# rosariocannavo/testudo

Hardware: AMD Instinct MI355X
Metric: PST commit+open sec, 2^20-var poly BLS12-377; G1 MSM Mscalar/s at 1/2/4/8 GPU (higher is better)
Workload: dtype u32; 1 GPU; single BLS12-377 G1 Pippenger MSM, 2^20 points per GPU (BASELINE configs[1]); n_points=1048576, curve=BLS12-377 G1, window_bits=16, parallelism=1 GPU

## Files before the change

### testudo_amd/csrc/msm_batch.hip

```cpp
#include "msm_sort.h"
#include "msm_acc.h"
#include "msm_reduce.h"

namespace tpst {

__global__ void __launch_bounds__(64, 1) k_build_tables(const uint32_t* __restrict__ bases, size_t N, int c, int W, uint32_t* __restrict__ table) {
  const size_t j = (size_t)blockIdx.x * blockDim.x + threadIdx.x;
  if (j >= N) return;
  G1A p = load_affine<Fq>(bases, j);
  for (int w = 0; w < W; w++) {
    store_rec29(table, (size_t)w * N + j, p);
    if (w + 1 < W) {
      Xyzz<Fq> x = to_xyzz(p);
      for (int i = 0; i < c; i++) x = dbl(x);
      p = to_affine(x);
    }
  }
}

hipError_t batch_tables_build(hipStream_t s, const uint32_t* d_bases, size_t N, int c, BatchTables& t) {
  batch_tables_free(t);
  t.N = N;
  t.c = c;
  t.W = num_windows(c);
  TPST_TRY(hipMalloc(&t.d_table, (size_t)t.W * N * REC29_WORDS * sizeof(uint32_t)));
  k_build_tables<<<grid_for(N, 64), 64, 0, s>>>(d_bases, N, c, t.W, t.d_table);
  return hipGetLastError();
}

void batch_tables_free(BatchTables& t) {
  if (t.d_table) (void)hipFree(t.d_table);
  t.d_table = nullptr;
  t.N = 0;
}

__device__ __forceinline__ void zero_bucket(uint4* zb, size_t key) {
  constexpr int Q = sizeof(Xyzz<Fq>) / 16;
#pragma unroll
  for (int i = 0; i < Q; i++) zb[key * Q + i] = make_uint4(0, 0, 0, 0);
}

__global__ void __launch_bounds__(256) k_batch_sort(const uint32_t* __restrict__ scalars, size_t rows, size_t N,
                                                    size_t row_stride, size_t col_stride, int c, int W,
                                                    uint32_t* __restrict__ keys, uint32_t* __restrict__ entries,
                                                    uint32_t* __restrict__ bstart, uint32_t* __restrict__ bend,
                                                    uint4* __restrict__ zb) {
  extern __shared__ uint32_t cnt[];
  const size_t nblk = gridDim.x;
  size_t r = blockIdx.x;
  if (nblk % 8 == 0) r = (blockIdx.x % 8) * (nblk / 8) + blockIdx.x / 8;
  if (r >= rows) return;
  const uint32_t nb = 1u << (c - 1);
  for (uint32_t b = threadIdx.x; b < nb; b += blockDim.x) cnt[b] = 0;
  __syncthreads();
  for (size_t j = threadIdx.x; j < N; j += blockDim.x) {
    uint32_t s[8];
    load_scalar(scalars + 8 * (r * row_stride + j * col_stride), s);
    uint32_t carry = 0;
    for (int w = 0; w < W; w++) {
      const int d = signed_digit(s, 8, w, c, W, carry);
      if (d) atomicAdd(&cnt[abs(d) - 1], 1u);
    }
  }
  __syncthreads();
  __shared__ uint32_t part[256];
  __shared__ uint32_t total_sh;
  const uint32_t per = (nb + blockDim.x - 1) / blockDim.x;
  const uint32_t b0 = threadIdx.x * per;
  uint32_t local = 0;
  for (uint32_t b = b0; b < b0 + per && b < nb; b++) local += cnt[b];
  part[threadIdx.x] = local;
  __syncthreads();
  if (threadIdx.x == 0) {
    uint32_t run = 0;
    for (unsigned t = 0; t < blockDim.x; t++) {
      const uint32_t v = part[t];
      part[t] = run;
      run += v;
    }
    total_sh = run;
  }
  __syncthreads();
  const size_t rowbase = r * N * (size_t)W;
  uint32_t run = part[threadIdx.x];
  for (uint32_t b = b0; b < b0 + per && b < nb; b++) {
    const uint32_t v = cnt[b];
    if (!v) zero_bucket(zb, r * nb + b);
    bstart[r * nb + b] = (uint32_t)(rowbase + run);
    bend[r * nb + b] = (uint32_t)(rowbase + run + v);
    cnt[b] = run;
    run += v;
  }
  __syncthreads();
  for (size_t j = threadIdx.x; j < N; j += blockDim.x) {
    uint32_t s[8];
    load_scalar(scalars + 8 * (r * row_stride + j * col_stride), s);
    uint32_t carry = 0;
    for (int w = 0; w < W; w++) {
      const int d = signed_digit(s, 8, w, c, W, carry);
      if (d) {
        const uint32_t b = (uint32_t)abs(d) - 1;
        const uint32_t pos = atomicAdd(&cnt[b], 1u);
        keys[rowbase + pos] = (uint32_t)(r * nb + b);
        entries[rowbase + pos] = (uint32_t)(w * N + j) | (d < 0 ? 0x80000000u : 0u);
      }
    }
  }
  const uint32_t total = total_sh;
  const uint32_t sent = (uint32_t)(rows * nb);
  for (size_t e = total + threadIdx.x; e < N * (size_t)W; e += blockDim.x) keys[rowbase + e] = sent;
}

constexpr int SB_THREADS = 1024;
constexpr int SB_SPT = 4;
constexpr uint32_t SB_NB = 2048;
constexpr uint32_t SB_STAGE = 15 * 1024;

template <int WC, int CC = 12>
__global__ void __launch_bounds__(SB_THREADS) k_batch_sort_staged(const uint32_t* __restrict__ scalars, size_t rows,
                                                                 size_t N, size_t row_stride, size_t col_stride, int c,
                                                                 int W, uint32_t* __restrict__ keys,
                                                                 uint32_t* __restrict__ entries,
                                                                 uint32_t* __restrict__ bstart,
                                                                 uint32_t* __restrict__ bend,
                                                                 uint4* __restrict__ zb) {
  __shared__ uint32_t start[SB_NB + 1];
  __shared__ uint32_t cur[SB_NB];
  __shared__ uint2 stage[SB_STAGE];
  __shared__ uint32_t part[SB_THREADS / 64];
  __shared__ uint32_t pass_lo, pass_hi;
  const size_t nblk = gridDim.x;
  size_t r = blockIdx.x;
  if (nblk % 8 == 0) r = (blockIdx.x % 8) * (nblk / 8) + blockIdx.x / 8;
  if (r >= rows) return;
  const uint32_t nb = 1u << (c - 1);
  const int tid = threadIdx.x;
  for (uint32_t b = tid; b < nb; b += SB_THREADS) cur[b] = 0;
  __syncthreads();
  for (int k = 0; k < SB_SPT; k++) {
    const size_t j = (size_t)tid + (size_t)k * SB_THREADS;
    if (j >= N) break;
    uint32_t sc[8];
    load_scalar(scalars + 8 * (r * row_stride + j * col_stride), sc);
    uint32_t carry = 0;
    if constexpr (WC > 0) {
#pragma unroll
      for (int w = 0; w < WC; w++) {
        const int d = signed_digit(sc, 8, w, CC, WC, carry);
        if (d) atomicAdd(&cur[abs(d) - 1], 1u);
      }
    } else {
      for (int w = 0; w < W; w++) {
        const int d = signed_digit(sc, 8, w, c, W, carry);
        if (d) atomicAdd(&cur[abs(d) - 1], 1u);
      }
    }
  }
  __syncthreads();
  {
    const uint32_t per = (nb + SB_THREADS - 1) / SB_THREADS;
    const uint32_t b0 = tid * per;
    uint32_t local = 0;
    for (uint32_t b = b0; b < b0 + per && b < nb; b++) local += cur[b];
    const int lane = tid & 63, wv = tid >> 6;
    uint32_t incl = local;
    for (int o = 1; o < 64; o <<= 1) {
      const uint32_t v = __shfl_up(incl, o, 64);
      if (lane >= o) incl += v;
    }
    if (lane == 63) part[wv] = incl;
    __syncthreads();
    if (tid == 0) {
      uint32_t run = 0;
      for (int i = 0; i < SB_THREADS / 64; i++) {
        const uint32_t v = part[i];
        part[i] = run;
        run += v;
      }
      start[nb] = run;
    }
    __syncthreads();
    uint32_t run = part[wv] + incl - local;
    for (uint32_t b = b0; b < b0 + per && b < nb; b++) {
      const uint32_t v = cur[b];
      start[b] = run;
      run += v;
    }
  }
  __syncthreads();
  const size_t rowbase = r * N * (size_t)W;
  for (uint32_t b = tid; b < nb; b += SB_THREADS) {
    if (start[b + 1] == start[b]) zero_bucket(zb, r * nb + b);
    bstart[r * nb + b] = (uint32_t)(rowbase + start[b]);
    bend[r * nb + b] = (uint32_t)(rowbase + start[b + 1]);
    cur[b] = start[b];
  }
  const uint32_t total = start[nb];
  if (tid == 0) pass_hi = 0;
  __syncthreads();
  for (;;) {
    if (tid == 0) {
      const uint32_t lo = pass_hi;
      uint32_t hi = lo;
      if (lo < nb) {
        const uint32_t lim = start[lo] + SB_STAGE;
        uint32_t a = lo + 1, z = nb;
        while (a < z) {
          const uint32_t m = (a + z + 1) >> 1;
          if (start[m] <= lim) a = m; else z = m - 1;
        }
        hi = a;
      }
      pass_lo = lo;
      pass_hi = hi;
    }
    __syncthreads();
    const uint32_t lo = pass_lo, hi = pass_hi;
    if (lo >= nb) break;
    const uint32_t p0 = start[lo], cnt = start[hi] - p0;
    const bool direct = cnt > SB_STAGE;
    auto place = [&](int d, int w, size_t j) {
      if (!d) return;
      const uint32_t b = (uint32_t)abs(d) - 1;
      if (b < lo || b >= hi) return;
      const uint32_t pos = atomicAdd(&cur[b], 1u);
      const uint2 e = make_uint2((uint32_t)(r * nb + b), (uint32_t)(w * N + j) | (d < 0 ? 0x80000000u : 0u));
      if (direct) {
        keys[rowbase + pos] = e.x;
        entries[rowbase + pos] = e.y;
      } else {
        stage[pos - p0] = e;
      }
    };
    for (int k = 0; k < SB_SPT; k++) {
      const size_t j = (size_t)tid + (size_t)k * SB_THREADS;
      if (j >= N) break;
      uint32_t sc[8];
      load_scalar(scalars + 8 * (r * row_stride + j * col_stride), sc);
      uint32_t carry = 0;
      if constexpr (WC > 0) {
#pragma unroll
        for (int w = 0; w < WC; w++) place(signed_digit(sc, 8, w, CC, WC, carry), w, j);
      } else {
        for (int w = 0; w < W; w++) place(signed_digit(sc, 8, w, c, W, carry), w, j);
      }
    }
    __syncthreads();
    if (!direct) {
      for (uint32_t i = tid; i < cnt; i += SB_THREADS) {
        const uint2 e = stage[i];
        keys[rowbase + p0 + i] = e.x;
        entries[rowbase + p0 + i] = e.y;
      }
    }
    __syncthreads();
  }
  const uint32_t sent = (uint32_t)(rows * nb);
  for (size_t e = total + tid; e < N * (size_t)W; e += SB_THREADS) keys[rowbase + e] = sent;
}

hipError_t msm_batch(Arena& ar, hipStream_t s, const BatchTables& t, const uint32_t* d_scalars, size_t rows,
                     size_t row_stride, size_t col_stride, Xyzz<Fq>* d_out) {
  if (rows == 0) return hipSuccess;
  const int c = t.c, W = t.W;
  const size_t N = t.N;
  const uint32_t nb = 1u << (c - 1);
  const size_t m = rows * N * (size_t)W;
  if (m >= (1ull << 32)) return hipErrorInvalidValue;
  const size_t nbk = rows * nb;
  static const size_t k1_threads = (size_t)4 * 64 * device_simds();
  int lg = 5;
  while (lg < 8 && (m >> (lg + 1)) >= k1_threads) lg++;
  const size_t nchunk = (m + ((size_t)1 << lg) - 1) >> lg;
  const size_t nblk = (nchunk + ACC_BLOCK - 1) / ACC_BLOCK;
  size_t need = 2 * Arena::need(m, 4) + 2 * Arena::need(nbk, 4) + Arena::need(nbk, sizeof(Xyzz<Fq>)) +
                Arena::need(nchunk, sizeof(Xyzz<Fq>)) + Arena::need(nblk, sizeof(Xyzz<Fq>)) +
                reduce_scratch<Fq>(rows, nb) + (red2_ok(nb) ? reduce2_scratch<Fq>(rows, nb) : 0) + 4096;
  ar.reset();
  TPST_TRY(ar.reserve(need));
  uint32_t* keys = ar.take<uint32_t>(m);
  uint32_t* entries = ar.take<uint32_t>(m);
  Xyzz<Fq>* part = ar.take<Xyzz<Fq>>(nchunk);
  Xyzz<Fq>* bpart = ar.take<Xyzz<Fq>>(nblk);
  uint32_t* bstart = ar.take<uint32_t>(nbk);
  uint32_t* bend = ar.take<uint32_t>(nbk);
  Xyzz<Fq>* buckets = ar.take<Xyzz<Fq>>(nbk);
  const unsigned nrow_blk = (unsigned)rows;
  Profiler* pf = ar.prof;
  Profiler dummy;
  if (!pf) pf = &dummy;
  pf->begin(ST_BATCH_SORT, s);
  if (N <= (size_t)SB_THREADS * SB_SPT && c == 12 && W == 22)
    k_batch_sort_staged<22, 12><<<nrow_blk, SB_THREADS, 0, s>>>(d_scalars, rows, N, row_stride, col_stride, c, W, keys,
                                                                 entries, bstart, bend, reinterpret_cast<uint4*>(buckets));
  else if (N <= (size_t)SB_THREADS * SB_SPT && c == 11 && W == 24)
    k_batch_sort_staged<24, 11><<<nrow_blk, SB_THREADS, 0, s>>>(d_scalars, rows, N, row_stride, col_stride, c, W, keys,
                                                                 entries, bstart, bend, reinterpret_cast<uint4*>(buckets));
  else if (N <= (size_t)SB_THREADS * SB_SPT && nb <= SB_NB)
    k_batch_sort_staged<0><<<nrow_blk, SB_THREADS, 0, s>>>(d_scalars, rows, N, row_stride, col_stride, c, W, keys,
                                                            entries, bstart, bend, reinterpret_cast<uint4*>(buckets));
  else
    k_batch_sort<<<nrow_blk, 256, nb * sizeof(uint32_t), s>>>(d_scalars, rows, N, row_stride, col_stride, c, W, keys,
                                                          entries, bstart, bend, reinterpret_cast<uint4*>(buckets));
  TPST_TRY(hipGetLastError());
  pf->end(ST_BATCH_SORT, s);
  pf->begin(ST_BUCKET_ACC, s);
  k_bucket_acc_chunk_lds<TPST_K1_MINW><<<(unsigned)nblk, ACC_BLOCK, 0, s>>>(keys, entries, m, nullptr, (uint32_t)nbk, bstart, bend,
                                                                  t.d_table, lg, buckets, part, bpart);
  TPST_TRY(hipGetLastError());
  k_bucket_fixup<Fq><<<grid_for(nblk, 64), 64, 0, s>>>(keys, m, nullptr, (uint32_t)nbk, bstart, bend, lg, nblk,
                                                       part, bpart, buckets);
  TPST_TRY(hipGetLastError());
  pf->end(ST_BUCKET_ACC, s);
  pf->begin(ST_REDUCE, s);
  if (red2_ok(nb))
    TPST_TRY(reduce_buckets2<Fq>(ar, s, buckets, rows, nb, d_out, 0));
  else
    TPST_TRY(reduce_buckets<Fq>(ar, s, buckets, rows, nb, d_out));
  pf->end(ST_REDUCE, s);
  return hipSuccess;
}

}
```

### testudo_amd/csrc/msm_reduce.h

```cpp
#pragma once
#include "msm_common.h"

namespace tpst {

template <bool PK, class F>
__device__ __forceinline__ Xyzz<typename AccField<F>::T> load_in(const Xyzz<F>* p, size_t i) {
  if constexpr (PK)
    return load_pk(p, i);
  else
    return load_acc(p, i);
}

template <class F, bool PK>
__global__ void __launch_bounds__(64) k_seg_reduce_quad(const Xyzz<F>* __restrict__ buckets, uint32_t nb, uint32_t L,
                                                        size_t nseg, Xyzz<F>* __restrict__ seg_out, int prio = 0) {
  using C = typename AccField<F>::T;
  set_wave_prio(prio);
  const size_t t = ((size_t)blockIdx.x * blockDim.x + threadIdx.x) >> 2;
  const int qi = threadIdx.x & 3;
  if (t >= nseg) return;
  const uint32_t S = nb / L;
  const size_t g = t / S;
  const uint32_t k = (uint32_t)(t % S);
  const size_t base = g * nb + (size_t)k * L;
  Xyzz<C> acc = Xyzz<C>::inf(), sum = Xyzz<C>::inf();
  for (int b = (int)L - 1; b >= 0; b--) {
    acc = add_quad(acc, load_in<PK>(buckets, base + b), qi);
    sum = add_quad(sum, acc, qi);
  }
  const uint32_t s0 = k * L;
  if (s0 != 0 && !is_inf(acc)) sum = add_quad(sum, scalar_mul_quad(acc, s0, 32 - __builtin_clz(s0), qi), qi);
  if (qi == 0) store_acc(seg_out, t, sum);
}

template <class F, bool PK>
__global__ void __launch_bounds__(64) k_seg_reduce_lane(const Xyzz<F>* __restrict__ buckets, uint32_t nb, uint32_t L,
                                                        size_t nseg, Xyzz<F>* __restrict__ seg_out) {
  using C = typename AccField<F>::T;
  const size_t t = (size_t)blockIdx.x * blockDim.x + threadIdx.x;
  if (t >= nseg) return;
  const uint32_t S = nb / L;
  const size_t g = t / S;
  const uint32_t k = (uint32_t)(t % S);
  const size_t base = g * nb + (size_t)k * L;
  Xyzz<C> acc = Xyzz<C>::inf(), sum = Xyzz<C>::inf();
  for (int b = (int)L - 1; b >= 0; b--) {
    acc = add(acc, load_in<PK>(buckets, base + b));
    sum = add(sum, acc);
  }
  const uint32_t s0 = k * L;
  if (s0 != 0 && !is_inf(acc)) sum = add(sum, scalar_mul_xyzz(acc, &s0, 32 - __builtin_clz(s0)));
  store_acc(seg_out, t, sum);
}

template <class F, int BS>
__global__ void __launch_bounds__(BS) k_group_reduce_quad(const Xyzz<F>* __restrict__ seg, uint32_t S,
                                                          Xyzz<F>* __restrict__ out, int prio = 0) {
  using C = typename AccField<F>::T;
  set_wave_prio(prio);
  constexpr int Q = BS / 4;
  __shared__ Xyzz<C> sh[Q];
  const size_t g = blockIdx.x;
  const int quad = threadIdx.x >> 2, qi = threadIdx.x & 3;
  Xyzz<C> acc = Xyzz<C>::inf();
  for (uint32_t k = quad; k < S; k += Q) acc = add_quad(acc, load_acc(seg, g * S + k), qi);
  if (qi == 0) sh[quad] = acc;
  __syncthreads();
  for (int h = Q / 2; h > 0; h >>= 1) {
    if (quad < h) {
      const Xyzz<C> v = add_quad(sh[quad], sh[quad + h], qi);
      if (qi == 0) sh[quad] = v;
    }
    __syncthreads();
  }
  if (threadIdx.x == 0) store_acc(out, g, sh[0]);
}

template <class F>
static __global__ void __launch_bounds__(64, 1) k_window_chain(const Xyzz<F>* __restrict__ win, int wlo, int whi,
                                                              int c, const Xyzz<F>* __restrict__ extra, int nextra,
                                                              Xyzz<F>* __restrict__ out) {
  using C = typename AccField<F>::T;
  if (blockIdx.x != 0) return;
  __builtin_amdgcn_s_setprio(3);
  const int qi = threadIdx.x & 3;
  Xyzz<C> acc = load_acc(win, whi - 1);
  for (int w = whi - 2; w >= wlo; w--) {
    for (int i = 0; i < c; i++) acc = dbl_quad(acc, qi);
    acc = add_quad(acc, load_acc(win, w), qi);
  }
  for (int i = 0; i < c * wlo; i++) acc = dbl_quad(acc, qi);
  for (int k = 0; k < nextra; k++) acc = add_quad(acc, load_acc(extra, k), qi);
  if (threadIdx.x == 0) store_acc(out, 0, acc);
}

static uint32_t reduce_seg_len(size_t groups, uint32_t nb) {
  uint32_t L = 4;
  while (L < 32 && 2 * L <= nb && groups * (nb / (2 * L)) >= ((size_t)1 << 18)) L *= 2;
  return nb >= L ? L : nb;
}

template <class F>
static size_t reduce_scratch(size_t groups, uint32_t nb) {
  const uint32_t L = reduce_seg_len(groups, nb);
  const size_t nseg = groups * (nb / L);
  return Arena::need(nseg, sizeof(Xyzz<F>)) + Arena::need(nseg / 64 + groups + 1, sizeof(Xyzz<F>));
}

template <class F>
static hipError_t sum_groups(Arena& ar, hipStream_t s, const Xyzz<F>* in, size_t groups, uint32_t S, Xyzz<F>* out,
                             int prio) {
  if (S >= 256 && S % 64 == 0) {
    Xyzz<F>* mid = ar.take<Xyzz<F>>(groups * S / 64);
    k_group_reduce_quad<F, 256><<<(unsigned)(groups * S / 64), 256, 0, s>>>(in, 64, mid, prio);
    TPST_TRY(hipGetLastError());
    k_group_reduce_quad<F, 256><<<(unsigned)groups, 256, 0, s>>>(mid, S / 64, out, prio);
  } else {
    k_group_reduce_quad<F, 256><<<(unsigned)groups, 256, 0, s>>>(in, S, out, prio);
  }
  return hipGetLastError();
}

template <class F>
static hipError_t reduce_buckets(Arena& ar, hipStream_t s, const Xyzz<F>* d_buckets, size_t groups, uint32_t nb,
                                 Xyzz<F>* d_group_out, int prio = 0, bool pk = true) {
  const uint32_t L = reduce_seg_len(groups, nb);
  const uint32_t S = nb / L;
  const size_t nseg = groups * S;
  Xyzz<F>* seg = ar.take<Xyzz<F>>(nseg);
  if (std::is_same<F, Fq>::value && nseg >= ((size_t)1 << 18)) {
    if (pk)
      k_seg_reduce_lane<F, true><<<grid_for(nseg, 64), 64, 0, s>>>(d_buckets, nb, L, nseg, seg);
    else
      k_seg_reduce_lane<F, false><<<grid_for(nseg, 64), 64, 0, s>>>(d_buckets, nb, L, nseg, seg);
  } else if (pk) {
    k_seg_reduce_quad<F, true><<<grid_for(4 * nseg, 64), 64, 0, s>>>(d_buckets, nb, L, nseg, seg, prio);
  } else {
    k_seg_reduce_quad<F, false><<<grid_for(4 * nseg, 64), 64, 0, s>>>(d_buckets, nb, L, nseg, seg, prio);
  }
  TPST_TRY(hipGetLastError());
  return sum_groups<F>(ar, s, seg, groups, S, d_group_out, prio);
}

template <class F, bool PK = true>
__global__ void __launch_bounds__(64) k_seg_run_quad(const Xyzz<F>* __restrict__ buckets, uint32_t nb, uint32_t L,
                                                     size_t nseg, Xyzz<F>* __restrict__ S_out,
                                                     Xyzz<F>* __restrict__ Tn, int prio = 0) {
  using C = typename AccField<F>::T;
  set_wave_prio(prio);
  const size_t t = ((size_t)blockIdx.x * blockDim.x + threadIdx.x) >> 2;
  const int qi = threadIdx.x & 3;
  if (t >= nseg) return;
  const uint32_t S = nb / L;
  const size_t g = t / S;
  const uint32_t k = (uint32_t)(t % S);
  const size_t base = g * nb + (size_t)k * L;
  Xyzz<C> acc = Xyzz<C>::inf(), sum = Xyzz<C>::inf();
  for (int b = (int)L - 1; b >= 0; b--) {
    acc = add_quad(acc, load_in<PK>(buckets, base + b), qi);
    sum = add_quad(sum, acc, qi);
  }
  if (qi == 0) {
    store_acc(S_out, t, sum);
    store_acc(Tn, g * S + (k ? k - 1 : S - 1), k ? acc : Xyzz<C>::inf());
  }
}

template <class F, bool PK = true>
__global__ void __launch_bounds__(64) k_seg_run_lane(const Xyzz<F>* __restrict__ buckets, uint32_t nb, uint32_t L,
                                                     size_t nseg, Xyzz<F>* __restrict__ S_out,
                                                     Xyzz<F>* __restrict__ Tn) {
  using C = typename AccField<F>::T;
  const size_t t = (size_t)blockIdx.x * blockDim.x + threadIdx.x;
  if (t >= nseg) return;
  const uint32_t S = nb / L;
  const size_t g = t / S;
  const uint32_t k = (uint32_t)(t % S);
  const size_t base = g * nb + (size_t)k * L;
  Xyzz<C> acc = Xyzz<C>::inf(), sum = Xyzz<C>::inf();
  for (int b = (int)L - 1; b >= 0; b--) {
    acc = add(acc, load_in<PK>(buckets, base + b));
    sum = add(sum, acc);
  }
  store_acc(S_out, t, sum);
  store_acc(Tn, g * S + (k ? k - 1 : S - 1), k ? acc : Xyzz<C>::inf());
}

template <class F>
__global__ void __launch_bounds__(64) k_lift_add_quad(const Xyzz<F>* __restrict__ a, const Xyzz<F>* __restrict__ b,
                                                      int lg, size_t groups, Xyzz<F>* __restrict__ out,
                                                      int prio = 0) {
  using C = typename AccField<F>::T;
  set_wave_prio(prio);
  const size_t g = ((size_t)blockIdx.x * blockDim.x + threadIdx.x) >> 2;
  const int qi = threadIdx.x & 3;
  if (g >= groups) return;
  Xyzz<C> r = load_acc(b, g);
  for (int i = 0; i < lg; i++) r = dbl_quad(r, qi);
  r = add_quad(r, load_acc(a, g), qi);
  if (qi == 0) store_acc(out, g, r);
}

constexpr int RED2_LG = 4;

static bool red2_ok(uint32_t nb) { return nb >= (16u << RED2_LG); }

template <class F>
static size_t reduce2_scratch(size_t groups, uint32_t nb) {
  const uint32_t S1 = nb >> RED2_LG;
  return 2 * Arena::need(groups * S1, sizeof(Xyzz<F>)) + reduce_scratch<F>(groups, S1) +
         Arena::need(groups * S1 / 64 + 1, sizeof(Xyzz<F>)) + 2 * Arena::need(groups, sizeof(Xyzz<F>));
}

#ifndef TPST_RED2_LANE
#define TPST_RED2_LANE 1
#endif
template <class F>
static hipError_t reduce_buckets2(Arena& ar, hipStream_t s, const Xyzz<F>* d_buckets, size_t groups, uint32_t nb,
                                  Xyzz<F>* d_group_out, int prio, bool lane_ok = false) {
  const uint32_t L1 = 1u << RED2_LG, S1 = nb / L1;
  const size_t nseg = groups * S1;
  Xyzz<F>* Sk = ar.take<Xyzz<F>>(nseg);
  Xyzz<F>* Tn = ar.take<Xyzz<F>>(nseg);
  Xyzz<F>* R = ar.take<Xyzz<F>>(groups);
  Xyzz<F>* SS = ar.take<Xyzz<F>>(groups);
  if (std::is_same<F, Fq>::value && (nseg >= ((size_t)1 << 18) || (TPST_RED2_LANE && lane_ok)))
    k_seg_run_lane<F><<<grid_for(nseg, 64), 64, 0, s>>>(d_buckets, nb, L1, nseg, Sk, Tn);
  else
    k_seg_run_quad<F><<<grid_for(4 * nseg, 64), 64, 0, s>>>(d_buckets, nb, L1, nseg, Sk, Tn, prio);
  TPST_TRY(hipGetLastError());
  TPST_TRY(reduce_buckets<F>(ar, s, Tn, groups, S1, R, prio, false));
  TPST_TRY(sum_groups<F>(ar, s, Sk, groups, S1, SS, prio));
  k_lift_add_quad<F><<<grid_for(4 * groups, 64), 64, 0, s>>>(SS, R, RED2_LG, groups, d_group_out, prio);
  return hipGetLastError();
}

}
```

Baseline: 329.0 Mscalar/s.

## Fuse two-level bucket reduce tail and pick lane/quad reduce by occupancy

Adds a single kernel that completes the two-level bucket reduction per group (running sums, doubling lift, and tree combine in shared memory). It replaces the chained segment-reduce, group-sum and lift-add launches. The lane vs quad choice and the first-level segment length are now derived from device SIMD count and wave occupancy, with env overrides and tracing. This cuts launch count and intermediate traffic in the reduce stage, but puts each group on one small block, which may serialize work when there are few groups.

```diff
diff --git a/testudo_amd/csrc/msm_batch.hip b/testudo_amd/csrc/msm_batch.hip
--- a/testudo_amd/csrc/msm_batch.hip
+++ b/testudo_amd/csrc/msm_batch.hip
@@ -1,3 +1,5 @@
+#include <cstdio>
+#include <cstring>
 #include "msm_sort.h"
 #include "msm_acc.h"
 #include "msm_reduce.h"
@@ -259,6 +261,49 @@
   for (size_t e = total + tid; e < N * (size_t)W; e += SB_THREADS) keys[rowbase + e] = sent;
 }
 
+struct CommitReduceMode {
+  int level1 = 0;
+  int tail = 0;
+};
+static const CommitReduceMode& commit_reduce_mode() {
+  static const CommitReduceMode mode = [] {
+    CommitReduceMode m;
+    const char* e = getenv("TPST_COMMIT_REDUCE");
+    if (!e) return m;
+    if (strstr(e, "quad")) m.level1 = 1;
+    if (strstr(e, "lane")) m.level1 = 2;
+    if (strstr(e, "chain")) m.tail = 1;
+    if (strstr(e, "fused")) m.tail = 2;
+    return m;
+  }();
+  return mode;
+}
+
+constexpr int SEG_RUN_QUAD_WPS = 2, SEG_REDUCE_QUAD_WPS = 1;
+
+struct CommitReducePlan {
+  bool two_level, lane, fused;
+  int lg;
+};
+static CommitReducePlan commit_reduce_plan(size_t rows, uint32_t nb) {
+  static const size_t simds = device_simds();
+  const CommitReduceMode& m = commit_reduce_mode();
+  CommitReducePlan p;
+  p.two_level = red2_ok(nb);
+  const size_t nseg = rows * (p.two_level ? nb >> RED2_LG : nb / reduce_seg_len(rows, nb));
+  const size_t quad_waves = 4 * nseg / 64;
+  const size_t slots = (size_t)(p.two_level ? SEG_RUN_QUAD_WPS : SEG_REDUCE_QUAD_WPS) * simds;
+  p.lane = m.level1 ? m.level1 == 2 : quad_waves >= slots;
+  p.fused = p.two_level && m.tail != 1;
+  p.lg = red2_seg_lg(p.lane, rows, nb, simds);
+  static const bool trace = getenv("TPST_COMMIT_REDUCE_TRACE") != nullptr;
+  if (trace)
+    fprintf(stderr, "commit reduce rows=%zu nb=%u level1=%s tail=%s L1=%u simds=%zu quad_wps=%zu\n", rows, nb,
+            p.lane ? "lane" : "quad", !p.two_level ? "single" : p.fused ? "fused" : "chain",
+            p.two_level ? 1u << p.lg : reduce_seg_len(rows, nb), simds, slots / simds);
+  return p;
+}
+
 hipError_t msm_batch(Arena& ar, hipStream_t s, const BatchTables& t, const uint32_t* d_scalars, size_t rows,
                      size_t row_stride, size_t col_stride, Xyzz<Fq>* d_out) {
   if (rows == 0) return hipSuccess;
@@ -273,9 +318,10 @@
   while (lg < 8 && (m >> (lg + 1)) >= k1_threads) lg++;
   const size_t nchunk = (m + ((size_t)1 << lg) - 1) >> lg;
   const size_t nblk = (nchunk + ACC_BLOCK - 1) / ACC_BLOCK;
+  const CommitReducePlan rp = commit_reduce_plan(rows, nb);
   size_t need = 2 * Arena::need(m, 4) + 2 * Arena::need(nbk, 4) + Arena::need(nbk, sizeof(Xyzz<Fq>)) +
                 Arena::need(nchunk, sizeof(Xyzz<Fq>)) + Arena::need(nblk, sizeof(Xyzz<Fq>)) +
-                reduce_scratch<Fq>(rows, nb) + (red2_ok(nb) ? reduce2_scratch<Fq>(rows, nb) : 0) + 4096;
+                reduce_scratch<Fq>(rows, nb) + (rp.two_level ? reduce2_scratch<Fq>(rows, nb, rp.lg) : 0) + 4096;
   ar.reset();
   TPST_TRY(ar.reserve(need));
   uint32_t* keys = ar.take<uint32_t>(m);
@@ -313,10 +359,10 @@
   TPST_TRY(hipGetLastError());
   pf->end(ST_BUCKET_ACC, s);
   pf->begin(ST_REDUCE, s);
-  if (red2_ok(nb))
-    TPST_TRY(reduce_buckets2<Fq>(ar, s, buckets, rows, nb, d_out, 0));
+  if (rp.two_level)
+    TPST_TRY((reduce_buckets2<Fq, true>(ar, s, buckets, rows, nb, d_out, 0, rp.lane, rp.lg, rp.fused)));
   else
-    TPST_TRY(reduce_buckets<Fq>(ar, s, buckets, rows, nb, d_out));
+    TPST_TRY(reduce_buckets<Fq>(ar, s, buckets, rows, nb, d_out, 0, true, rp.lane));
   pf->end(ST_REDUCE, s);
   return hipSuccess;
 }
diff --git a/testudo_amd/csrc/msm_reduce.h b/testudo_amd/csrc/msm_reduce.h
--- a/testudo_amd/csrc/msm_reduce.h
+++ b/testudo_amd/csrc/msm_reduce.h
@@ -123,12 +123,12 @@
 
 template <class F>
 static hipError_t reduce_buckets(Arena& ar, hipStream_t s, const Xyzz<F>* d_buckets, size_t groups, uint32_t nb,
-                                 Xyzz<F>* d_group_out, int prio = 0, bool pk = true) {
+                                 Xyzz<F>* d_group_out, int prio = 0, bool pk = true, int lane = -1) {
   const uint32_t L = reduce_seg_len(groups, nb);
   const uint32_t S = nb / L;
   const size_t nseg = groups * S;
   Xyzz<F>* seg = ar.take<Xyzz<F>>(nseg);
-  if (std::is_same<F, Fq>::value && nseg >= ((size_t)1 << 18)) {
+  if (std::is_same<F, Fq>::value && (lane < 0 ? nseg >= ((size_t)1 << 18) : lane != 0)) {
     if (pk)
       k_seg_reduce_lane<F, true><<<grid_for(nseg, 64), 64, 0, s>>>(d_buckets, nb, L, nseg, seg);
     else
@@ -201,37 +201,109 @@
   if (qi == 0) store_acc(out, g, r);
 }
 
+template <class F, int BS>
+__global__ void __launch_bounds__(BS) k_red2_tail(const Xyzz<F>* __restrict__ Sk, const Xyzz<F>* __restrict__ Tn,
+                                                  uint32_t S1, int lg, Xyzz<F>* __restrict__ out, int prio = 0) {
+  using C = typename AccField<F>::T;
+  set_wave_prio(prio);
+  constexpr int Q = BS / 4;
+  __shared__ Xyzz<C> sh[2][Q], own[Q];
+  const size_t g = blockIdx.x;
+  const int quad = threadIdx.x >> 2, qi = threadIdx.x & 3;
+  const uint32_t per = S1 > (uint32_t)Q ? S1 / Q : 1;
+  const uint32_t lo = (uint32_t)quad * per;
+  {
+    Xyzz<C> A = Xyzz<C>::inf(), r = Xyzz<C>::inf();
+    if (lo < S1) {
+      for (int j = (int)per - 1; j >= 0; j--) {
+        A = add_quad(A, load_acc(Tn, g * S1 + lo + j), qi);
+        r = add_quad(r, A, qi);
+      }
+      for (int i = 0; i < lg; i++) r = dbl_quad(r, qi);
+      for (uint32_t j = 0; j < per; j++) r = add_quad(r, load_acc(Sk, g * S1 + lo + j), qi);
+    }
+    if (qi == 0) {
+      sh[0][quad] = A;
+      own[quad] = r;
+    }
+  }
+  __syncthreads();
+  Xyzz<C>*cur = sh[0], *nxt = sh[1];
+  for (int d = 1; d < Q; d <<= 1) {
+    if (quad + d < Q) {
+      const Xyzz<C> v = add_quad(cur[quad], cur[quad + d], qi);
+      if (qi == 0) nxt[quad] = v;
+    } else if (qi == 0) {
+      nxt[quad] = cur[quad];
+    }
+    __syncthreads();
+    Xyzz<C>* t = cur;
+    cur = nxt;
+    nxt = t;
+  }
+  if (quad + 1 < Q) {
+    const Xyzz<C> u = cur[quad + 1], mine = own[quad];
+    Xyzz<C> r = u;
+    for (uint32_t p = per << lg; p > 1; p >>= 1) r = dbl_quad(r, qi);
+    r = add_quad(r, mine, qi);
+    if (qi == 0) own[quad] = r;
+  }
+  __syncthreads();
+  for (int h = Q / 2; h > 0; h >>= 1) {
+    if (quad < h) {
+      const Xyzz<C> v = add_quad(own[quad], own[quad + h], qi);
+      if (qi == 0) own[quad] = v;
+    }
+    __syncthreads();
+  }
+  if (threadIdx.x == 0) store_acc(out, g, own[0]);
+}
+
 constexpr int RED2_LG = 4;
 
+constexpr int RED2_LANE_WPS = 2;
+static int red2_seg_lg(bool lane_rows, size_t groups, uint32_t nb, size_t simds) {
+  int lg = RED2_LG;
+  if (lane_rows)
+    while (lg > 3 && ((groups * nb) >> lg) < (size_t)RED2_LANE_WPS * 64 * simds) lg--;
+  return lg;
+}
+
 static bool red2_ok(uint32_t nb) { return nb >= (16u << RED2_LG); }
 
 template <class F>
-static size_t reduce2_scratch(size_t groups, uint32_t nb) {
-  const uint32_t S1 = nb >> RED2_LG;
+static size_t reduce2_scratch(size_t groups, uint32_t nb, int lg = RED2_LG) {
+  const uint32_t S1 = nb >> lg;
   return 2 * Arena::need(groups * S1, sizeof(Xyzz<F>)) + reduce_scratch<F>(groups, S1) +
          Arena::need(groups * S1 / 64 + 1, sizeof(Xyzz<F>)) + 2 * Arena::need(groups, sizeof(Xyzz<F>));
 }
 
-#ifndef TPST_RED2_LANE
-#define TPST_RED2_LANE 1
-#endif
-template <class F>
+constexpr int RED2_TAIL_BS = 64;
+
+template <class F, bool TAIL = false>
 static hipError_t reduce_buckets2(Arena& ar, hipStream_t s, const Xyzz<F>* d_buckets, size_t groups, uint32_t nb,
-                                  Xyzz<F>* d_group_out, int prio, bool lane_ok = false) {
-  const uint32_t L1 = 1u << RED2_LG, S1 = nb / L1;
+                                  Xyzz<F>* d_group_out, int prio, bool lane = false, int lg = RED2_LG,
+                                  bool fused = false) {
+  const uint32_t L1 = 1u << lg, S1 = nb / L1;
   const size_t nseg = groups * S1;
   Xyzz<F>* Sk = ar.take<Xyzz<F>>(nseg);
   Xyzz<F>* Tn = ar.take<Xyzz<F>>(nseg);
   Xyzz<F>* R = ar.take<Xyzz<F>>(groups);
   Xyzz<F>* SS = ar.take<Xyzz<F>>(groups);
-  if (std::is_same<F, Fq>::value && (nseg >= ((size_t)1 << 18) || (TPST_RED2_LANE && lane_ok)))
+  if (std::is_same<F, Fq>::value && lane)
     k_seg_run_lane<F><<<grid_for(nseg, 64), 64, 0, s>>>(d_buckets, nb, L1, nseg, Sk, Tn);
   else
     k_seg_run_quad<F><<<grid_for(4 * nseg, 64), 64, 0, s>>>(d_buckets, nb, L1, nseg, Sk, Tn, prio);
   TPST_TRY(hipGetLastError());
+  if constexpr (TAIL) {
+    if (fused) {
+      k_red2_tail<F, RED2_TAIL_BS><<<(unsigned)groups, RED2_TAIL_BS, 0, s>>>(Sk, Tn, S1, lg, d_group_out, prio);
+      return hipGetLastError();
+    }
+  }
   TPST_TRY(reduce_buckets<F>(ar, s, Tn, groups, S1, R, prio, false));
   TPST_TRY(sum_groups<F>(ar, s, Sk, groups, S1, SS, prio));
-  k_lift_add_quad<F><<<grid_for(4 * groups, 64), 64, 0, s>>>(SS, R, RED2_LG, groups, d_group_out, prio);
+  k_lift_add_quad<F><<<grid_for(4 * groups, 64), 64, 0, s>>>(SS, R, lg, groups, d_group_out, prio);
   return hipGetLastError();
 }
 
```

Result: no change. 328.8 Mscalar/s (median of 2 runs) (-0.1%).
